# GuildOfWeavers/distaff

Measured on NVIDIA H100. Metric: prove ms for 2^20-step trace (default 120-bit ProofOptions), lower is better.
Workload: dtype u128 (128-bit prime field) + u32 (blake3)

## Files before the change

### distaff_b200/csrc/ntt.cu

```cuda
#define DG_MUL_CALL 1
#include "ntt_pass.cuh"

namespace dg {

PassKernel pass_kernel_inline(bool lane_major, int log_l, int rmax, int bt);
template <bool LM, int RMAX, int BT, int MINB> static PassKernel pass_kernel_t(int log_l) {
    switch (log_l) {
        case 1: return ntt_pass_kernel<1, LM, RMAX, BT, MINB, 0>;  case 2: return ntt_pass_kernel<2, LM, RMAX, BT, MINB, 0>;
        case 3: return ntt_pass_kernel<3, LM, RMAX, BT, MINB, 0>;  case 4: return ntt_pass_kernel<4, LM, RMAX, BT, MINB, 0>;
        case 5: return ntt_pass_kernel<5, LM, RMAX, BT, MINB, 0>;  case 6: return ntt_pass_kernel<6, LM, RMAX, BT, MINB, 0>;
        case 7: return ntt_pass_kernel<7, LM, RMAX, BT, MINB, 0>;  case 8: return ntt_pass_kernel<8, LM, RMAX, BT, MINB, 0>;
        case 9: return ntt_pass_kernel<9, LM, RMAX, BT, MINB, 0>;  case 10: return ntt_pass_kernel<10, LM, RMAX, BT, MINB, 0>;
    }
    throw Error(-1, "unsupported sub-transform size");
}

struct PassCfg { int rmax, bt, inl; };
struct NttConfig { PassCfg a, b, af; int tile_log; };
static PassCfg parse_cfg(const char *env, PassCfg d) {
    const char *e = getenv(env);
    if (e) { int r = 0, t = 0, i = 0; if (sscanf(e, "%d,%d,%d", &r, &t, &i) == 3) d = PassCfg{r, t, i}; }
    if (d.rmax < 2 || d.rmax > 4) d.rmax = 4;
    if (d.bt != 512 && d.bt != 1024) d.bt = 256;
    return d;
}
static const NttConfig &ntt_config() {
    static NttConfig cfg;
    static bool init = false;
    if (!init) {
        cfg.a = parse_cfg("DG_NTT_A", PassCfg{3, 512, 1});
        cfg.b = parse_cfg("DG_NTT_B", PassCfg{3, 512, 1});
        cfg.af = parse_cfg("DG_NTT_AF", PassCfg{2, 512, 1});
        const char *e = getenv("DG_NTT_TILE");
        cfg.tile_log = e ? atoi(e) : 12;
        if (cfg.tile_log < 12 || cfg.tile_log > 13) cfg.tile_log = 12;
        init = true;
    }
    return cfg;
}

static void launch_pass(Context &c, int log_l, PassGeom g, const fe *src, fe *dst, unsigned blocks_x, unsigned by, unsigned bz) {
    const int L = 1 << log_l, T = 1 << g.log_t;
    const size_t data = g.lane_major ? (size_t)T * (L + (L >> 3) + 1) : (size_t)L * T;
    const size_t smem = ((size_t)L + data) * sizeof(fe);
    const NttConfig &nc = ntt_config();
    const PassCfg cfg = g.lane_major ? nc.b : ((g.coset_on && !g.coset_fast) ? nc.af : nc.a);
    int rmax = cfg.rmax, bt = cfg.bt;
    PassKernel k = nullptr;
    if (cfg.inl) k = pass_kernel_inline(g.lane_major != 0, log_l, rmax, bt);
    if (!k) {
        const bool lm = g.lane_major != 0;
        if (bt == 1024) bt = 512;
        if (rmax == 4) { bt = 256; k = lm ? pass_kernel_t<true, 4, 256, 2>(log_l) : pass_kernel_t<false, 4, 256, 2>(log_l); }
        else if (rmax == 3 && bt == 512) k = lm ? pass_kernel_t<true, 3, 512, 2>(log_l) : pass_kernel_t<false, 3, 512, 2>(log_l);
        else if (rmax == 3) k = lm ? pass_kernel_t<true, 3, 256, 3>(log_l) : pass_kernel_t<false, 3, 256, 3>(log_l);
        else if (bt == 512) k = lm ? pass_kernel_t<true, 2, 512, 2>(log_l) : pass_kernel_t<false, 2, 512, 2>(log_l);
        else k = lm ? pass_kernel_t<true, 2, 256, 4>(log_l) : pass_kernel_t<false, 2, 256, 4>(log_l);
    }
    int threads = (L * T) >> (log_l < rmax ? log_l : rmax);
    if (threads > bt) threads = bt;
    if (threads < 32) threads = 32;
    set_func_smem(c, (const void *)k, 200 * 1024);
    DG_REQUIRE(by <= 65535 && bz <= 65535, "batch too large for one launch");
    k<<<dim3(blocks_x, by, bz), threads, smem, c.stream>>>(src, dst, g); c.launches++;
    DG_CUDA(cudaGetLastError());
}

static int lanes_log(int log_l, long long available) {
    int lt = 4;
    const int tile = 1 << ntt_config().tile_log;
    while ((1 << (log_l + lt)) > tile && lt > 0) lt--;
    while ((1LL << lt) > available && lt > 0) lt--;
    return lt;
}

static int split_passes(int log_n, int l[3]) {
    if (log_n <= MAX_LOG_L) { l[0] = log_n; return 1; }
    if (log_n <= 2 * MAX_LOG_L) { l[0] = (log_n + 1) / 2; l[1] = log_n / 2; return 2; }
    DG_REQUIRE(log_n <= 3 * MAX_LOG_L, "transform too large");
    l[0] = (log_n + 2) / 3; l[1] = (log_n + 1) / 3; l[2] = log_n / 3;
    return 3;
}

struct CosetSpec { bool on; int log_blowup; int fold; unsigned coset0; };

__global__ void lde_twiddle_fill_kernel(fe *table, TwiddleRef cw, int log_n, int log_r1, int log_b) {
    const unsigned long long i = (unsigned long long)blockIdx.x * blockDim.x + threadIdx.x;
    if (i >> (log_n + log_b)) return;
    const unsigned long long c = i >> log_n, pos = i & ((1ULL << log_n) - 1);
    const unsigned long long lane = pos & ((1ULL << log_r1) - 1), k = pos >> log_r1;
    table[i] = tw_lookup(cw, lane * ((k << log_b) + c));
}
static const fe *lde_twiddle_table(Context &c, int log_n, int log_b, int l0) {
    static long long cap = -1;
    if (cap < 0) { const char *e = getenv("DG_LDE_TW_MB"); cap = (e ? atoll(e) : 1024) << 20; }
    const size_t bytes = ((size_t)16 << (log_n + log_b));
    if ((long long)bytes > cap) return nullptr;
    const long long key = ((long long)log_n << 16) | (log_b << 8) | l0;
    auto it = c.lde_twiddles.find(key);
    if (it == c.lde_twiddles.end()) {
        DevBuf t;
        t.alloc(bytes, true);
        const unsigned long long cnt = 1ULL << (log_n + log_b);
        lde_twiddle_fill_kernel<<<(unsigned)((cnt + 255) / 256), 256, 0, c.stream>>>(t.as<fe>(), c.twiddle(log_n + log_b, false), log_n, log_n - l0, log_b);
        c.launches++;
        DG_CUDA(cudaGetLastError());
        it = c.lde_twiddles.emplace(key, std::move(t)).first;
    }
    return it->second.as<fe>();
}

static void run_transform(Context &c, const fe *src, fe *dst, int log_n, bool inverse, unsigned by, unsigned bz, long long src_stride_z,
                          long long dst_stride_y, long long dst_stride_z, CosetSpec cs) {
    int l[3];
    const int np = split_passes(log_n, l);
    const long long n = 1LL << log_n;
    fe scale = fe_make(1, 0);
    if (inverse) scale = host_inv(fe_make((unsigned long long)n, 0));

    PassGeom base;
    memset(&base, 0, sizeof base);
    if (cs.on) {
        base.coset_on = 1;
        base.fold = cs.fold;
        base.fold_stride = n;
        base.cw = c.twiddle(log_n + cs.log_blowup, false);
        base.log_blowup = cs.log_blowup;
        base.coset0 = cs.coset0;
        if (cs.fold == 1) {
            const int log_order = l[0] + cs.log_blowup;
            base.coset_fast = 1;
            base.cw_point = c.single_table(log_order);
            base.cw_point_mask = (1u << log_order) - 1u;
        }
    }

    fe *tmp = nullptr;
    long long tmp_stride_y = n, tmp_stride_z = n * by;
    if (np > 1) {
        c.ntt_tmp.ensure((size_t)n * by * bz * sizeof(fe), true);
        tmp = c.ntt_tmp.as<fe>();
// ... 31 lines not shown
        const long long N3 = 1LL << l[2];
        PassGeom g;
        memset(&g, 0, sizeof g);
        g.log_t = lanes_log(l[1], N3);
        g.num_tiles = (unsigned)(N3 >> g.log_t);
        g.in_point = N3; g.in_lane = 1; g.in_outer = R1; g.out_point = N3; g.out_lane = 1; g.out_outer = R1;
        g.in_batch_y = tmp_stride_y; g.in_batch_z = tmp_stride_z; g.out_batch_y = tmp_stride_y; g.out_batch_z = tmp_stride_z;
        g.lane_major = 0;
        g.tw_on = 1; g.tw = c.twiddle(log_n - l[0], inverse);
        g.roots = c.roots(l[1], inverse);
        launch_pass(c, l[1], g, tmp, tmp, (unsigned)(g.num_tiles * N1), by, bz);
    }
    {
        const int ll = l[np - 1];
        PassGeom g;
        memset(&g, 0, sizeof g);
        g.log_t = lanes_log(ll, N1);
        g.num_tiles = (unsigned)(N1 >> g.log_t);
        g.in_point = 1; g.in_lane = R1; g.in_outer = (np == 3) ? (1LL << ll) : 0;
        g.out_lane = 1; g.out_outer = (np == 3) ? N1 : 0; g.out_point = N1 * N2;
        g.in_batch_y = tmp_stride_y; g.in_batch_z = tmp_stride_z; g.out_batch_y = dst_stride_y; g.out_batch_z = dst_stride_z;
        g.lane_major = 1; g.tw_on = 0;
        g.has_scale = inverse; g.scale = scale;
        g.roots = c.roots(ll, inverse);
        launch_pass(c, ll, g, tmp, dst, (unsigned)(g.num_tiles * N2), by, bz);
    }
}

void ntt_batch(Context &c, const fe *src, fe *dst, int log_n, int batch, size_t src_stride, size_t dst_stride, bool inverse) {
    DG_REQUIRE(log_n >= 1 && log_n <= 30, "log_n out of range");
    const size_t n = (size_t)1 << log_n;
    size_t max_chunk = std::max<size_t>(1, ((size_t)1 << 30) / (n * sizeof(fe)));
    if (max_chunk > 65535) max_chunk = 65535;
    for (size_t b0 = 0; b0 < (size_t)batch; b0 += max_chunk) {
        size_t nb = std::min(max_chunk, (size_t)batch - b0);
        run_transform(c, src + b0 * src_stride, dst + b0 * dst_stride, log_n, inverse, 1, (unsigned)nb, (long long)src_stride, 0,
                      (long long)dst_stride, CosetSpec{false, 0, 1, 0});
    }
}

__global__ void __launch_bounds__(256) prefold8_kernel(const fe *__restrict__ src, fe *__restrict__ dst, int log_n, int log_b, const fe *__restrict__ zeta,
                                                       TwiddleRef twN, fe w8, fe w8_2, fe w8_3) {
    const unsigned long long n = 1ULL << log_n;
    const unsigned long long t = (unsigned long long)blockIdx.x * blockDim.x + threadIdx.x;
    if (t >> (log_n + log_b - 3)) return;
    const unsigned long long j = t & (n - 1);
    const unsigned r = (unsigned)(t >> log_n);
    const unsigned bmask = (1u << log_b) - 1u, step = 1u << (log_b - 3);
    fe x[8];
#pragma unroll
    for (int f = 0; f < 8; f++) x[f] = src[j + (unsigned long long)f * n];
    if (r) {
#pragma unroll
        for (int f = 1; f < 8; f++) x[f] = fe_mul(x[f], zeta[(r * (unsigned)f) & bmask]);
    }
    fe u[4], v[4];
    const fe wp[4] = {fe_make(1, 0), w8, w8_2, w8_3};
#pragma unroll
    for (int i = 0; i < 4; i++) {
        u[i] = fe_add(x[i], x[i + 4]);
        v[i] = fe_sub(x[i], x[i + 4]);
        if (i) v[i] = fe_mul(v[i], wp[i]);
    }
    fe X[8];
    {
        fe p0 = fe_add(u[0], u[2]), p1 = fe_add(u[1], u[3]), q0 = fe_sub(u[0], u[2]), q1 = fe_mul(fe_sub(u[1], u[3]), w8_2);
        X[0] = fe_add(p0, p1); X[4] = fe_sub(p0, p1); X[2] = fe_add(q0, q1); X[6] = fe_sub(q0, q1);
        p0 = fe_add(v[0], v[2]); p1 = fe_add(v[1], v[3]); q0 = fe_sub(v[0], v[2]); q1 = fe_mul(fe_sub(v[1], v[3]), w8_2);
        X[1] = fe_add(p0, p1); X[5] = fe_sub(p0, p1); X[3] = fe_add(q0, q1); X[7] = fe_sub(q0, q1);
    }
    fe cur = tw_lookup(twN, (unsigned long long)r * j);
    const fe rho = tw_lookup(twN, (unsigned long long)step * j);
#pragma unroll
    for (int q = 0; q < 8; q++) {
        dst[((unsigned long long)(step * (unsigned)q + r) << log_n) + j] = fe_mul(X[q], cur);
        if (q < 7) cur = fe_mul(cur, rho);
    }
}

void lde_batch(Context &c, const fe *src, fe *dst, int log_n, int log_blowup, int fold, int batch, size_t src_stride, size_t dst_stride,
               unsigned coset0, unsigned ncosets) {
    DG_REQUIRE(log_n >= 1 && log_n + log_blowup <= 30, "LDE domain too large");
    const size_t n = (size_t)1 << log_n;
    const unsigned cosets = ncosets ? ncosets : (1u << log_blowup);
    DG_REQUIRE(coset0 + cosets <= (1u << log_blowup), "coset range out of bounds");
    static int prefold = -1;
    if (prefold < 0) { const char *e = getenv("DG_LDE_PREFOLD"); prefold = e ? atoi(e) : 1; }
    if (prefold && fold == 8 && batch == 1 && cosets == (1u << log_blowup) && log_blowup >= 3 && log_blowup <= 8) {
        DevBuf pre((size_t)n * cosets * sizeof(fe));
        const fe w8 = host_root_of_unity(3), w8_2 = fe_mul(w8, w8);
        const unsigned long long threads = (unsigned long long)n << (log_blowup - 3);
        prefold8_kernel<<<(unsigned)((threads + 255) / 256), 256, 0, c.stream>>>(src, pre.as<fe>(), log_n, log_blowup, c.single_table(log_blowup),
                                                                                 c.twiddle(log_n + log_blowup, false), w8, w8_2, fe_mul(w8_2, w8)); c.launches++;
        DG_CUDA(cudaGetLastError());
        ntt_batch(c, pre.as<fe>(), dst, log_n, (int)cosets, n, n, false);
        return;
    }
    static size_t scratch_cap = 0;
    if (!scratch_cap) { const char *e = getenv("DG_NTT_SCRATCH_MB"); scratch_cap = (size_t)(e ? atoll(e) : 4096) << 20; }
    size_t max_chunk = std::max<size_t>(1, scratch_cap / (n * cosets * sizeof(fe)));
    if (max_chunk > 65535) max_chunk = 65535;
    for (size_t b0 = 0; b0 < (size_t)batch; b0 += max_chunk) {
        size_t nb = std::min(max_chunk, (size_t)batch - b0);
        run_transform(c, src + b0 * src_stride, dst + b0 * dst_stride, log_n, false, cosets, (unsigned)nb, (long long)src_stride,
                      (long long)n, (long long)dst_stride, CosetSpec{true, log_blowup, fold, coset0});
    }
}

}
```

### distaff_b200/csrc/ntt_inl.cu

```cuda
#include "ntt_pass.cuh"

namespace dg {

template <bool LM, int RMAX, int BT, int MINB> static PassKernel inl_t(int log_l) {
    switch (log_l) {
        case 8: return ntt_pass_kernel<8, LM, RMAX, BT, MINB, 1>;
        case 9: return ntt_pass_kernel<9, LM, RMAX, BT, MINB, 1>;
        case 10: return ntt_pass_kernel<10, LM, RMAX, BT, MINB, 1>;
    }
    return nullptr;
}

PassKernel pass_kernel_inline(bool lm, int log_l, int rmax, int bt) {
    if (rmax == 3 && bt == 1024) return lm ? inl_t<true, 3, 1024, 1>(log_l) : inl_t<false, 3, 1024, 1>(log_l);
    if (rmax == 3 && bt == 512) return lm ? inl_t<true, 3, 512, 2>(log_l) : inl_t<false, 3, 512, 2>(log_l);
    if (rmax == 3) return lm ? inl_t<true, 3, 256, 3>(log_l) : inl_t<false, 3, 256, 3>(log_l);
    if (rmax == 2 && bt == 512) return lm ? inl_t<true, 2, 512, 2>(log_l) : inl_t<false, 2, 512, 2>(log_l);
    if (rmax == 2) return lm ? inl_t<true, 2, 256, 4>(log_l) : inl_t<false, 2, 256, 4>(log_l);
    return nullptr;
}

}
```

### distaff_b200/csrc/ntt_pass.cuh

```cuda
#pragma once
#include "common.cuh"

namespace dg {

struct PassGeom {
    int log_t;
    unsigned num_tiles;
    long long in_outer, in_lane, in_point;
    long long out_outer, out_lane, out_point;
    long long in_batch_y, out_batch_y, in_batch_z, out_batch_z;
    int lane_major;
    int tw_on;
    TwiddleRef tw;
    int has_scale;
    fe scale;
    int coset_on;
    int fold;
    long long fold_stride;
    TwiddleRef cw;
    int coset_fast;
    const fe *cw_point;
    unsigned cw_point_mask;
    const fe *tw_full;
    long long tw_full_stride;
    int log_blowup;
    unsigned coset0;
    const fe *roots;
};

__device__ __forceinline__ fe tw_lookup(const TwiddleRef &t, unsigned long long e) {
    unsigned ee = (unsigned)e & t.mask;
    fe a = t.lo[ee & ((1u << t.lo_bits) - 1u)];
    fe b = t.hi[ee >> t.lo_bits];
    return fe_mul(a, b);
}

template <int LOG_L, int S0, int RHO>
__device__ __forceinline__ void dif_regs(fe *x, const fe *s_tw, int g_lo) {
    constexpr int L = 1 << LOG_L, R = 1 << RHO;
    constexpr int LOG_SP = LOG_L - S0 - RHO;
#pragma unroll
    for (int u = 0; u < RHO; u++) {
        const int hr = R >> (u + 1);
        const int st = S0 + u;
        const fe *W = s_tw + (L - (L >> st));
#pragma unroll
        for (int i = 0; i < R; i++) {
            if ((i & hr) == 0) {
                fe a = x[i], b = x[i + hr];
                x[i] = fe_add(a, b);
                fe d = fe_sub(a, b);
                if (st != LOG_L - 1 && !(LOG_SP == 0 && (i & (hr - 1)) == 0)) d = fe_mul(d, W[g_lo + ((i & (hr - 1)) << LOG_SP)]);
                x[i + hr] = d;
            }
        }
    }
}

template <int LOG_L, bool LANE_MAJOR>
__device__ __forceinline__ int sidx(int pos, int t, int T) {
    constexpr int L = 1 << LOG_L;
    constexpr int LS = L + (L >> 3) + 1;
    return LANE_MAJOR ? (t * LS + pos + (pos >> 3)) : (pos * T + t);
}

template <int LOG_L, int S0, int RHO, bool FIRST, bool LAST, bool LANE_MAJOR>
__device__ __forceinline__ void ntt_round(const fe *__restrict__ src, fe *__restrict__ dst, fe *s_data, const fe *s_tw, const PassGeom &g,
                                          unsigned tile, long long in_base) {
    constexpr int L = 1 << LOG_L, R = 1 << RHO;
    constexpr int LOG_B = LOG_L - S0, LOG_SP = LOG_B - RHO;
    constexpr int N_GLO = 1 << LOG_SP, N_GHI = 1 << S0;
    const int T = 1 << g.log_t;
    const int units = (L >> RHO) * T;
    for (int u = threadIdx.x; u < units; u += blockDim.x) {
        int t, g_lo, g_hi;
        if (!LANE_MAJOR || LAST) {
            t = u & (T - 1);
            const int rest = u >> g.log_t;
            g_lo = rest & (N_GLO - 1);
            g_hi = rest >> LOG_SP;
        } else {
            g_lo = u & (N_GLO - 1);
            const int rest = u >> LOG_SP;
            g_hi = rest & (N_GHI - 1);
            t = rest >> S0;
        }
        const int gbase = (g_hi << LOG_B) + g_lo;
        fe x[R];
#pragma unroll
        for (int m = 0; m < R; m++) {
            const int pos = gbase + (m << LOG_SP);
            if (FIRST) {
                const long long j = in_base + (long long)t * g.in_lane + (long long)pos * g.in_point;
                if (g.coset_fast) {
                    x[m] = fe_mul(src[j], g.cw_point[((g.coset0 + (unsigned)blockIdx.y) * (unsigned)pos) & g.cw_point_mask]);
                } else if (g.coset_on) {
                    const unsigned long long c = g.coset0 + blockIdx.y;
                    const fe u = tw_lookup(g.cw, c * (unsigned long long)g.fold_stride);
                    fe v = src[j + (long long)(g.fold - 1) * g.fold_stride];
                    for (int f = g.fold - 2; f >= 0; f--) v = fe_add(fe_mul(v, u), src[j + (long long)f * g.fold_stride]);
                    x[m] = fe_mul(v, tw_lookup(g.cw, c * (unsigned long long)j));
                } else {
                    x[m] = src[j];
                }
            } else {
                x[m] = s_data[sidx<LOG_L, LANE_MAJOR>(pos, t, T)];
            }
        }
        dif_regs<LOG_L, S0, RHO>(x, s_tw, g_lo);
#pragma unroll
        for (int m = 0; m < R; m++) {
            const int pos = gbase + (m << LOG_SP);
            if (LAST) {
                const unsigned k = __brev((unsigned)pos) >> (32 - LOG_L);
                fe v = x[m];
                if (g.coset_fast && g.tw_on) {
                    if (g.tw_full)
                        v = fe_mul(v, g.tw_full[(long long)(g.coset0 + blockIdx.y) * g.tw_full_stride + (long long)(tile * T + t) * g.out_lane + (long long)k * g.out_point]);
                    else
                        v = fe_mul(v, tw_lookup(g.cw, (unsigned long long)(tile * T + t) * (((unsigned long long)k << g.log_blowup) + g.coset0 + blockIdx.y)));
                }
                else if (g.tw_on) v = fe_mul(v, tw_lookup(g.tw, (unsigned long long)(tile * T + t) * k));
                if (g.has_scale) v = fe_mul(v, g.scale);
                dst[(long long)t * g.out_lane + (long long)k * g.out_point] = v;
            } else {
                s_data[sidx<LOG_L, LANE_MAJOR>(pos, t, T)] = x[m];
            }
        }
    }
}

template <int LOG_L, int RMAX, int S0, bool LANE_MAJOR>
__device__ __forceinline__ void ntt_rounds(const fe *__restrict__ src, fe *__restrict__ dst, fe *s_data, const fe *s_tw, const PassGeom &g,
                                           unsigned tile, long long in_base) {
    constexpr int REM = LOG_L - S0, LEFT = (REM + RMAX - 1) / RMAX, RHO = (REM + LEFT - 1) / LEFT;
    ntt_round<LOG_L, S0, RHO, S0 == 0, S0 + RHO == LOG_L, LANE_MAJOR>(src, dst, s_data, s_tw, g, tile, in_base);
    if constexpr (S0 + RHO < LOG_L) {
        __syncthreads();
        ntt_rounds<LOG_L, RMAX, S0 + RHO, LANE_MAJOR>(src, dst, s_data, s_tw, g, tile, in_base);
    }
}

template <int LOG_L, bool LANE_MAJOR, int RMAX, int BT, int MINB, int TAG>
__global__ void __launch_bounds__(BT, MINB) ntt_pass_kernel(const fe *__restrict__ src, fe *__restrict__ dst, const PassGeom g) {
    extern __shared__ __align__(16) unsigned char smem_raw[];
    constexpr int L = 1 << LOG_L;
    fe *s_tw = reinterpret_cast<fe *>(smem_raw);
    fe *s_data = s_tw + L;
    const int T = 1 << g.log_t;
    const unsigned tile = blockIdx.x % g.num_tiles, outer = blockIdx.x / g.num_tiles;
    const long long in_base = (long long)outer * g.in_outer + (long long)tile * T * g.in_lane;
    src += (long long)blockIdx.y * g.in_batch_y + (long long)blockIdx.z * g.in_batch_z;
    dst += (long long)blockIdx.y * g.out_batch_y + (long long)blockIdx.z * g.out_batch_z + (long long)outer * g.out_outer +
           (long long)tile * T * g.out_lane;
    for (int i = threadIdx.x; i < L - 1; i += blockDim.x) s_tw[i] = g.roots[i];
    if (g.tw_full) {
        const fe *tb = g.tw_full + (long long)(g.coset0 + blockIdx.y) * g.tw_full_stride + (long long)tile * T * g.out_lane;
        for (int k = threadIdx.x; k < L; k += blockDim.x)
            asm volatile("prefetch.global.L2 [%0];" :: "l"(tb + (long long)k * g.out_point));
    }
    __syncthreads();
    ntt_rounds<LOG_L, RMAX, 0, LANE_MAJOR>(src, dst, s_data, s_tw, g, tile, in_base);
}

typedef void (*PassKernel)(const fe *, fe *, const PassGeom);

}
```

### distaff_b200/csrc/prover.cu

```cuda
#include "prover.h"
#include "air.h"
#include "host_fs.h"
#include "poly.h"
#include "shard.h"
#include <array>
#include <atomic>
#include <memory>
#include <thread>

namespace dg {

namespace {

struct StageClock {
    cudaStream_t s;
    cudaEvent_t ev[10];
    explicit StageClock(cudaStream_t stream) : s(stream) { for (auto &e : ev) DG_CUDA(cudaEventCreate(&e)); }
    ~StageClock() { for (auto &e : ev) cudaEventDestroy(e); }
    void mark(int i) { DG_CUDA(cudaEventRecord(ev[i], s)); }
    float between(int a, int b) { float ms = 0; cudaEventElapsedTime(&ms, ev[a], ev[b]); return ms; }
};

struct SubClock {
    bool on;
    cudaStream_t s;
    std::vector<std::pair<std::string, cudaEvent_t>> marks;
    explicit SubClock(cudaStream_t stream) : on(getenv("DG_SUBSTAGE") != nullptr), s(stream) {}
    void mark(const char *name) {
        if (!on) return;
        cudaEvent_t e;
        cudaEventCreate(&e);
        cudaEventRecord(e, s);
        marks.emplace_back(name, e);
    }
    void report(int rank) {
        if (!on) return;
        cudaStreamSynchronize(s);
        std::string line = "SUBSTAGE rank " + std::to_string(rank) + ":";
        for (size_t i = 1; i < marks.size(); i++) {
            float ms = 0;
            cudaEventElapsedTime(&ms, marks[i - 1].second, marks[i].second);
            char buf[96];
            snprintf(buf, sizeof buf, " %s=%.3f", marks[i].first.c_str(), ms);
            line += buf;
        }
        if (rank == 0 || atoi(getenv("DG_SUBSTAGE")) >= 2) fprintf(stderr, "%s\n", line.c_str());
        for (auto &m : marks) cudaEventDestroy(m.second);
        marks.clear();
    }
};

void d2h(Context &c, void *dst, const void *src, size_t bytes) {
    DG_CUDA(cudaMemcpyAsync(dst, src, bytes, cudaMemcpyDeviceToHost, c.stream));
    DG_CUDA(cudaStreamSynchronize(c.stream));
}
void h2d(Context &c, void *dst, const void *src, size_t bytes) {
    DG_CUDA(cudaMemcpyAsync(dst, src, bytes, cudaMemcpyHostToDevice, c.stream));
}

void debug_dump(Context &c, const char *name, const void *dev, size_t bytes) {
    const char *dir = getenv("DG_DEBUG_DUMP");
    if (!dir) return;
    std::vector<uint8_t> host(bytes);
    d2h(c, host.data(), dev, bytes);
    std::string path = std::string(dir) + "/" + name + ".bin";
    FILE *f = fopen(path.c_str(), "wb");
    if (!f) return;
    fwrite(host.data(), 1, bytes, f);
    fclose(f);
}

void debug_dump_host(const char *name, const void *host, size_t bytes) {
    const char *dir = getenv("DG_DEBUG_DUMP");
    if (!dir) return;
    std::string path = std::string(dir) + "/" + name + ".bin";
    FILE *f = fopen(path.c_str(), "wb");
    if (!f) return;
    fwrite(host, 1, bytes, f);
    fclose(f);
}


void write_digest_vec(fs::ByteWriter &w, const std::vector<Digest> &v) {
    w.u64(v.size());
    for (auto &d : v) w.raw(d.data(), 32);
}
void write_digest_vv(fs::ByteWriter &w, const std::vector<std::vector<Digest>> &v) {
    w.u64(v.size());
    for (auto &x : v) write_digest_vec(w, x);
}
void write_felt_vec(fs::ByteWriter &w, const std::vector<fe> &v) {
    w.u64(v.size());
    for (auto &x : v) w.felt(x);
}

int ilog2(uint64_t v) { int l = 0; while ((1ULL << l) < v) l++; return l; }

struct FriLayerDev {
    DevBuf leaves, nodes, folded;
    const fe *vals;
    Layout layout;
    bool sharded = false;
    ShardedTree tree;
    Digest root;
};

}

class TraceUploader {
public:
    static const int WORKERS = 4, SLOTS = 2;
    TraceUploader(Context &c, fe *d_regs, const uint8_t *const *host_cols, int w, uint64_t n, const std::vector<int> &bounds)
        : c_(c), w_(w), bounds_(bounds), nchunks_((int)bounds.size() - 1), col_bytes_(n * 16), done_(nchunks_, nullptr), recorded_(nchunks_) {
        for (auto &r : recorded_) r.store(0);
        for (auto &e : done_) DG_CUDA(cudaEventCreateWithFlags(&e, cudaEventDisableTiming));
        cudaEvent_t ready;
        DG_CUDA(cudaEventCreateWithFlags(&ready, cudaEventDisableTiming));
        DG_CUDA(cudaEventRecord(ready, c.stream));
        cudaPointerAttributes attr;
        bool pinned = cudaPointerGetAttributes(&attr, host_cols[0]) == cudaSuccess && attr.type != cudaMemoryTypeUnregistered;
        cudaGetLastError();
        if (getenv("DG_NO_STAGING")) pinned = true;
        if (pinned) {
            DG_CUDA(cudaStreamWaitEvent(c.copy_stream, ready, 0));
            for (int i = 0; i < nchunks_; i++) {
                for (int j = bounds_[i]; j < bounds_[i + 1]; j++)
                    DG_CUDA(cudaMemcpyAsync(d_regs + (size_t)j * n, host_cols[j], col_bytes_, cudaMemcpyHostToDevice, c.copy_stream));
                DG_CUDA(cudaEventRecord(done_[i], c.copy_stream));
                recorded_[i].store(1);
            }
        } else {
            c.staging.ensure((size_t)WORKERS * SLOTS * col_bytes_);
            for (int t = 0; t < WORKERS; t++) {
                if (!c.staging_streams[t]) DG_CUDA(cudaStreamCreateWithFlags(&c.staging_streams[t], cudaStreamNonBlocking));
                DG_CUDA(cudaStreamWaitEvent(c.staging_streams[t], ready, 0));
            }
            const int dev = c.device;
            for (int t = 0; t < WORKERS; t++)
                workers_.emplace_back([this, t, dev, d_regs, host_cols, n]() {
                    cudaSetDevice(dev);
                    cudaStream_t st = c_.staging_streams[t];
                    cudaEvent_t slot_free[SLOTS] = {nullptr, nullptr};
                    int use = 0;
                    for (int i = t; i < nchunks_ && !failed_.load(); i += WORKERS) {
                        for (int j = bounds_[i]; j < bounds_[i + 1]; j++, use++) {
                            const int s = use % SLOTS;
                            uint8_t *slot = (uint8_t *)c_.staging.p + ((size_t)t * SLOTS + s) * col_bytes_;
                            if (slot_free[s]) cudaEventSynchronize(slot_free[s]);
                            else cudaEventCreateWithFlags(&slot_free[s], cudaEventDisableTiming);
                            memcpy(slot, host_cols[j], col_bytes_);
                            if (cudaMemcpyAsync(d_regs + (size_t)j * n, slot, col_bytes_, cudaMemcpyHostToDevice, st) != cudaSuccess) failed_.store(true);
                            cudaEventRecord(slot_free[s], st);
                        }
                        if (cudaEventRecord(done_[i], st) != cudaSuccess) failed_.store(true);
                        recorded_[i].store(1);
                    }
                    for (int i = t; i < nchunks_; i += WORKERS) recorded_[i].store(1);
                    cudaStreamSynchronize(st);
                    for (auto &e : slot_free) if (e) cudaEventDestroy(e);
                });
        }
        cudaEventDestroy(ready);
    }
    void wait_chunk(int i) {
        while (!recorded_[i].load()) std::this_thread::yield();
        if (failed_.load()) throw Error(DG_ERR_CUDA, "host trace upload failed");
        DG_CUDA(cudaStreamWaitEvent(c_.stream, done_[i], 0));
    }
    int chunks() const { return nchunks_; }
    ~TraceUploader() {
        failed_.store(true);
        for (auto &t : workers_) t.join();
        cudaStreamSynchronize(c_.copy_stream);
        for (auto &e : done_) if (e) cudaEventDestroy(e);
    }
private:
    Context &c_;
    int w_;
    std::vector<int> bounds_;
    int nchunks_;
    size_t col_bytes_;
    std::vector<cudaEvent_t> done_;
    std::vector<std::atomic<int>> recorded_;
    std::atomic<bool> failed_{false};
    std::vector<std::thread> workers_;
};

static Proof *prove_core(Context &c, fe *d_regs, const uint8_t *const *host_cols, uint32_t width, uint64_t length, uint32_t ctx_depth,
                         uint32_t loop_depth, const uint8_t *inputs16, uint32_t n_inputs, const uint8_t *outputs16, uint32_t n_outputs,
                         const dg_options_t &opt, dg_prove_stats_t *stats) {
    const uint64_t n = length, b = opt.extension_factor;
    DG_REQUIRE(opt.hash_id == 0, "unsupported hash function (only blake3 is serialisable, options.rs:107)");
    DG_REQUIRE(b >= 16 && b <= 256 && (b & (b - 1)) == 0, "extension_factor must be a power of 2 between 16 and 256");
    DG_REQUIRE(opt.num_queries > 0 && opt.num_queries <= 128, "num_queries must be in 1..128");
    DG_REQUIRE(opt.grinding_factor <= 32, "grinding factor cannot be greater than 32");
    DG_REQUIRE(n >= 16 && (n & (n - 1)) == 0, "execution trace length must be a power of 2 and at least 16");
    DG_REQUIRE(ctx_depth <= 16, "context depth cannot be greater than 16");
    DG_REQUIRE(loop_depth <= 8, "loop depth cannot be greater than 8");
    DG_REQUIRE(width < 128, "execution trace cannot have more than 128 registers");
    DG_REQUIRE(width > 15 + ctx_depth + loop_depth, "user stack must consist of at least one register");
    DG_REQUIRE(n_inputs <= 8 && n_outputs <= 8, "cannot have more than 8 public inputs / outputs");
    const int w = (int)width, log_n = ilog2(n), log_b = ilog2(b), log_N = log_n + log_b;
    DG_REQUIRE(log_N <= 30, "LDE domain too large");
    const uint64_t N = n * b, E = n * 8;
    const int stack_depth = w - 15 - (int)ctx_depth - (int)loop_depth;
    DG_REQUIRE(stack_depth <= 32, "stack depth cannot be greater than 32");
    std::vector<fe> inputs(n_inputs), outputs(n_outputs);
    if (n_inputs) memcpy(inputs.data(), inputs16, n_inputs * 16);
    if (n_outputs) memcpy(outputs.data(), outputs16, n_outputs * 16);

    ArenaScope arena_scope;
    StageClock clk(c.stream);
    SubClock sub(c.stream);
    if (sub.on) c.mark = [&sub](const char *name) { sub.mark(name); }; else c.mark = nullptr;
    struct MarkReset { Context &c; ~MarkReset() { c.mark = nullptr; } } mark_reset{c};
    const unsigned long long launches0 = c.launches;
    Proof *proof = new Proof();
    std::unique_ptr<Proof> guard(proof);

    const int G = c.world, g = c.rank;
    int log_g = 0;
    while ((1 << log_g) < G) log_g++;
    DG_REQUIRE((b >> log_g) >= 4 && G <= 8, "extension factor too small for this many GPUs (need >= 4 cosets per rank)");
    const int log_nc = log_b - log_g;
    const uint64_t nc = 1ULL << log_nc, N_loc = n * nc;
    const unsigned c0 = (unsigned)(g * nc);

    clk.mark(0);
    sub.mark("start");
    const int cpr = (w + G - 1) / G;
    auto col_count = [&](int r) { return w / G + (r < w % G ? 1 : 0); };
    auto col_start = [&](int r) { return r * (w / G) + std::min(r, w % G); };
    DevBuf polys((size_t)w * n * 16), ext((size_t)w * N_loc * 16);
    if (G == 1) {
        if (!host_cols) {
            ntt_batch(c, d_regs, polys.as<fe>(), log_n, w, n, n, true);
            lde_batch(c, polys.as<fe>(), ext.as<fe>(), log_n, log_b, 1, w, n, N_loc, c0, (unsigned)nc);
        } else {
            const int chunk = (int)std::max<uint64_t>(1, std::min<uint64_t>(w, ((uint64_t)1 << 26) / (n * 16)));
            std::vector<int> bounds = {0};
            for (int step = 1; bounds.back() < w; step = std::min(chunk, step * 2)) bounds.push_back(std::min(w, bounds.back() + step));
            TraceUploader up(c, d_regs, host_cols, w, n, bounds);
            for (int i = 0; i < up.chunks(); i++) {
                const int j0 = bounds[i], cols = bounds[i + 1] - j0;
                up.wait_chunk(i);
                ntt_batch(c, d_regs + (size_t)j0 * n, polys.as<fe>() + (size_t)j0 * n, log_n, cols, n, n, true);
                lde_batch(c, polys.as<fe>() + (size_t)j0 * n, ext.as<fe>() + (size_t)j0 * N_loc, log_n, log_b, 1, cols, n, N_loc, c0, (unsigned)nc);
            }
        }
    } else {
        const int j0 = col_start(g), mine = col_count(g);
        DevBuf own((size_t)cpr * n * 16), slots((size_t)cpr * G * n * 16);
        if (mine > 0) {
            if (host_cols) {
                std::vector<int> bounds(mine + 1);
                for (int i = 0; i <= mine; i++) bounds[i] = i;
                TraceUploader up(c, d_regs + (size_t)j0 * n, host_cols + j0, mine, n, bounds);
                for (int i = 0; i < up.chunks(); i++) {
                    up.wait_chunk(i);
                    ntt_batch(c, d_regs + (size_t)(j0 + i) * n, own.as<fe>() + (size_t)i * n, log_n, 1, n, n, true);
                }
            } else {
                ntt_batch(c, d_regs + (size_t)j0 * n, own.as<fe>(), log_n, mine, n, n, true);
            }
        }
    sub.mark("1.intt");
        cudaEvent_t ev_own, ev_all;
        DG_CUDA(cudaEventCreateWithFlags(&ev_own, cudaEventDisableTiming));
        DG_CUDA(cudaEventCreateWithFlags(&ev_all, cudaEventDisableTiming));
        DG_CUDA(cudaEventRecord(ev_own, c.stream));
        DG_CUDA(cudaStreamWaitEvent(c.comm_stream, ev_own, 0));
        comm_all_gather(c, own.p, slots.p, (size_t)cpr * n * 16, c.comm_stream);
        for (int r = 0; r < G; r++)
            if (col_count(r) > 0)
                DG_CUDA(cudaMemcpyAsync(polys.as<fe>() + (size_t)col_start(r) * n, slots.as<fe>() + (size_t)r * cpr * n, (size_t)col_count(r) * n * 16,
                                        cudaMemcpyDeviceToDevice, c.comm_stream));
        DG_CUDA(cudaEventRecord(ev_all, c.comm_stream));
        if (mine > 0) lde_batch(c, own.as<fe>(), ext.as<fe>() + (size_t)j0 * N_loc, log_n, log_b, 1, mine, n, N_loc, c0, (unsigned)nc);
    sub.mark("1.lde_own");
        DG_CUDA(cudaStreamWaitEvent(c.stream, ev_all, 0));
        if (j0 > 0) lde_batch(c, polys.as<fe>(), ext.as<fe>(), log_n, log_b, 1, j0, n, N_loc, c0, (unsigned)nc);
        if (j0 + mine < w)
            lde_batch(c, polys.as<fe>() + (size_t)(j0 + mine) * n, ext.as<fe>() + (size_t)(j0 + mine) * N_loc, log_n, log_b, 1, w - j0 - mine, n, N_loc, c0,
                      (unsigned)nc);
        cudaEventDestroy(ev_own);
        cudaEventDestroy(ev_all);
    }

    clk.mark(1);
    sub.mark("1.lde");
    DevBuf t_leaves(N_loc * 32);
    hash_trace_rows(c, ext.as<fe>(), t_leaves.p, w, log_n, log_nc);
    sub.mark("2.hash_rows");
    ShardedTree t_tree;
    t_tree.build(c, t_leaves.p, n, log_nc);
    memcpy(proof->trace_root, t_tree.root.data(), 32);

    clk.mark(2);
    sub.mark("2.tree");
    fe last_row[3];
    if (host_cols) {
        for (int j = 0; j < 3; j++) memcpy(&last_row[j], host_cols[j] + (n - 1) * 16, 16);
    } else {
        DevBuf d_last(48);
        for (int j = 0; j < 3; j++) DG_CUDA(cudaMemcpyAsync((uint8_t *)d_last.p + 16 * j, d_regs + (size_t)j * n + (n - 1), 16, cudaMemcpyDeviceToDevice, c.stream));
        d2h(c, last_row, d_last.p, 48);
    }
    const fe op_count = last_row[0];
    const fe program_hash[2] = {last_row[1], last_row[2]};
    fs::ConstraintCoefficients cc = fs::draw_constraint_coefficients(proof->trace_root, ctx_depth, loop_depth, stack_depth, inputs, outputs,
                                                                      op_count, program_hash);
    DevBuf &d_periodic = c.d_periodic;
    if (!d_periodic.p) {
        std::vector<fe> per = fs::periodic_tables();
        d_periodic.alloc(per.size() * 16, true);
        h2d(c, d_periodic.p, per.data(), per.size() * 16);
        DG_CUDA(cudaStreamSynchronize(c.stream));
    }
    const size_t T = cc.coefA.size(), nb = cc.bAi.size();
    DevBuf d_coef((2 * T + 4 * nb) * 16), d_violation(4);
    {
        std::vector<fe> pack;
        pack.insert(pack.end(), cc.coefA.begin(), cc.coefA.end());
        pack.insert(pack.end(), cc.coefB.begin(), cc.coefB.end());
        pack.insert(pack.end(), cc.bAi.begin(), cc.bAi.end());
        pack.insert(pack.end(), cc.bBi.begin(), cc.bBi.end());
        pack.insert(pack.end(), cc.bAf.begin(), cc.bAf.end());
        pack.insert(pack.end(), cc.bBf.begin(), cc.bBf.end());
        h2d(c, d_coef.p, pack.data(), pack.size() * 16);
        DG_CUDA(cudaStreamSynchronize(c.stream));
    }
    DG_CUDA(cudaMemsetAsync(d_violation.p, 0, 4, c.stream));
    DevBuf evals(3 * E * 16);
    {
        const int num_c8 = 8 >> log_g;
        const uint64_t E_loc = n * num_c8;
        DevBuf evals_loc(E_loc * 16), gathered(E * 16);
        AirParams P;
        memset(&P, 0, sizeof P);
        P.w = w; P.ctx_depth = ctx_depth; P.loop_depth = loop_depth; P.stack_depth = stack_depth;
        P.cl = std::max<int>(ctx_depth, 1); P.ll = std::max<int>(loop_depth, 1); P.sl = std::max(stack_depth, 8);
        P.log_n = log_n; P.log_blowup = log_b;
        P.ext = ext.as<fe>(); P.col_stride = N_loc;
        P.c8_base = g * num_c8; P.num_c8 = num_c8;
        P.t_ev = evals_loc.as<fe>();
        P.periodic = d_periodic.as<fe>();
        const fe *base = d_coef.as<fe>();
        P.coefA = base; P.coefB = base + T;
        P.twN = c.twiddle(log_N, false);
        static const int GROUP_DEG[6] = {2, 3, 4, 6, 7, 8};
        for (int gi = 0; gi < 6; gi++) P.inc[gi] = (8 * n - 1) - (n - 1) * GROUP_DEG[gi];
        P.violation = d_violation.as<unsigned>();
    sub.mark("3.setup");
        launch_constraint_eval(c, P);
    sub.mark("3.eval");
        comm_all_reduce_max_u32(c, d_violation.as<unsigned>(), 1);
        unsigned violation = 0;
        d2h(c, &violation, d_violation.p, 4);
        if (violation) throw Error(DG_ERR_UNSATISFIED, "transition constraints at step " + std::to_string(violation - 1) + " were not satisfied");
    sub.mark("3.violation_sync");
        ntt_batch(c, evals_loc.as<fe>(), evals_loc.as<fe>(), log_n, num_c8, n, n, true);
        comm_all_gather(c, evals_loc.as<fe>(), gathered.as<fe>(), E_loc * 16);
    sub.mark("3.intt+gather");
        coset_interp_finish(c, gathered.as<fe>(), evals.as<fe>() + 2 * E, log_n);
        boundary_coeffs(c, polys.as<fe>(), n, (int)nb, base + 2 * T, cc.KiA, cc.KiB, cc.KfA, cc.KfB, evals.as<fe>(), evals.as<fe>() + E);
    }
    debug_dump(c, "t_coeffs", evals.as<fe>() + 2 * E, E * 16);
// ... 316 lines not shown
```

Before: 134.2.

## Specialize NTT pass kernels by pass kind and reuse trace for coset zero

Replaces runtime branching on coset, twiddle and scale flags inside the NTT pass kernel with a compile-time PassKind template parameter, so each variant compiles only the multiply path it needs. It also changes the default radix for strided and contiguous passes from 3 to 2. When the LDE covers coset 0, the original trace columns are copied into the extension buffer instead of being recomputed by an NTT, which removes one coset of transforms. The cost is more kernel instantiations, and the copy assumes coset 0 of the extension equals the trace in natural order.

```diff
diff --git a/distaff_b200/csrc/ntt.cu b/distaff_b200/csrc/ntt.cu
--- a/distaff_b200/csrc/ntt.cu
+++ b/distaff_b200/csrc/ntt.cu
@@ -3,16 +3,20 @@
 
 namespace dg {
 
-PassKernel pass_kernel_inline(bool lane_major, int log_l, int rmax, int bt);
-template <bool LM, int RMAX, int BT, int MINB> static PassKernel pass_kernel_t(int log_l) {
-    switch (log_l) {
-        case 1: return ntt_pass_kernel<1, LM, RMAX, BT, MINB, 0>;  case 2: return ntt_pass_kernel<2, LM, RMAX, BT, MINB, 0>;
-        case 3: return ntt_pass_kernel<3, LM, RMAX, BT, MINB, 0>;  case 4: return ntt_pass_kernel<4, LM, RMAX, BT, MINB, 0>;
-        case 5: return ntt_pass_kernel<5, LM, RMAX, BT, MINB, 0>;  case 6: return ntt_pass_kernel<6, LM, RMAX, BT, MINB, 0>;
-        case 7: return ntt_pass_kernel<7, LM, RMAX, BT, MINB, 0>;  case 8: return ntt_pass_kernel<8, LM, RMAX, BT, MINB, 0>;
-        case 9: return ntt_pass_kernel<9, LM, RMAX, BT, MINB, 0>;  case 10: return ntt_pass_kernel<10, LM, RMAX, BT, MINB, 0>;
-    }
-    throw Error(-1, "unsupported sub-transform size");
+PassKernel pass_kernel_inline(int kind, int log_l, int rmax, int bt);
+
+static int pass_kind(const PassGeom &g) {
+    if (!g.lane_major) {
+        DG_REQUIRE(g.tw_on && !g.has_scale, "strided NTT pass without inter-pass twiddle");
+        if (g.coset_fast) return g.tw_full ? PK_COSET_TWFULL : PK_COSET_TW;
+        return g.coset_on ? PK_FOLD_TW : PK_TW;
+    }
+    DG_REQUIRE(!g.tw_on, "contiguous NTT pass with inter-pass twiddle");
+    if (g.coset_on) {
+        DG_REQUIRE(!g.has_scale, "scaled coset transform");
+        return g.coset_fast ? PK_COSET_ONE : PK_FOLD_ONE;
+    }
+    return g.has_scale ? PK_LAST_SCALE : PK_LAST;
 }
 
 struct PassCfg { int rmax, bt, inl; };
@@ -28,8 +32,8 @@
     static NttConfig cfg;
     static bool init = false;
     if (!init) {
-        cfg.a = parse_cfg("DG_NTT_A", PassCfg{3, 512, 1});
-        cfg.b = parse_cfg("DG_NTT_B", PassCfg{3, 512, 1});
+        cfg.a = parse_cfg("DG_NTT_A", PassCfg{2, 512, 1});
+        cfg.b = parse_cfg("DG_NTT_B", PassCfg{2, 512, 1});
         cfg.af = parse_cfg("DG_NTT_AF", PassCfg{2, 512, 1});
         const char *e = getenv("DG_NTT_TILE");
         cfg.tile_log = e ? atoi(e) : 12;
@@ -45,18 +49,19 @@
     const size_t smem = ((size_t)L + data) * sizeof(fe);
     const NttConfig &nc = ntt_config();
     const PassCfg cfg = g.lane_major ? nc.b : ((g.coset_on && !g.coset_fast) ? nc.af : nc.a);
+    const int kind = pass_kind(g);
     int rmax = cfg.rmax, bt = cfg.bt;
     PassKernel k = nullptr;
-    if (cfg.inl) k = pass_kernel_inline(g.lane_major != 0, log_l, rmax, bt);
+    if (cfg.inl) k = pass_kernel_inline(kind, log_l, rmax, bt);
     if (!k) {
-        const bool lm = g.lane_major != 0;
         if (bt == 1024) bt = 512;
-        if (rmax == 4) { bt = 256; k = lm ? pass_kernel_t<true, 4, 256, 2>(log_l) : pass_kernel_t<false, 4, 256, 2>(log_l); }
-        else if (rmax == 3 && bt == 512) k = lm ? pass_kernel_t<true, 3, 512, 2>(log_l) : pass_kernel_t<false, 3, 512, 2>(log_l);
-        else if (rmax == 3) k = lm ? pass_kernel_t<true, 3, 256, 3>(log_l) : pass_kernel_t<false, 3, 256, 3>(log_l);
-        else if (bt == 512) k = lm ? pass_kernel_t<true, 2, 512, 2>(log_l) : pass_kernel_t<false, 2, 512, 2>(log_l);
-        else k = lm ? pass_kernel_t<true, 2, 256, 4>(log_l) : pass_kernel_t<false, 2, 256, 4>(log_l);
-    }
+        if (rmax == 4) { bt = 256; k = pass_kernel_of<4, 256, 2, 0, 1, MAX_LOG_L>(kind, log_l); }
+        else if (rmax == 3 && bt == 512) k = pass_kernel_of<3, 512, 2, 0, 1, MAX_LOG_L>(kind, log_l);
+        else if (rmax == 3) k = pass_kernel_of<3, 256, 3, 0, 1, MAX_LOG_L>(kind, log_l);
+        else if (bt == 512) k = pass_kernel_of<2, 512, 2, 0, 1, MAX_LOG_L>(kind, log_l);
+        else k = pass_kernel_of<2, 256, 4, 0, 1, MAX_LOG_L>(kind, log_l);
+    }
+    DG_REQUIRE(k, "unsupported sub-transform size");
     int threads = (L * T) >> (log_l < rmax ? log_l : rmax);
     if (threads > bt) threads = bt;
     if (threads < 32) threads = 32;
@@ -254,8 +259,9 @@
                unsigned coset0, unsigned ncosets) {
     DG_REQUIRE(log_n >= 1 && log_n + log_blowup <= 30, "LDE domain too large");
     const size_t n = (size_t)1 << log_n;
-    const unsigned cosets = ncosets ? ncosets : (1u << log_blowup);
-    DG_REQUIRE(coset0 + cosets <= (1u << log_blowup), "coset range out of bounds");
+    DG_REQUIRE(log_blowup >= 0 && log_blowup <= 16 && fold >= 1, "bad LDE shape");
+    const unsigned b = 1u << log_blowup, cosets = ncosets ? ncosets : b;
+    DG_REQUIRE(coset0 < b && cosets <= b - coset0, "coset range out of bounds");
     static int prefold = -1;
     if (prefold < 0) { const char *e = getenv("DG_LDE_PREFOLD"); prefold = e ? atoi(e) : 1; }
     if (prefold && fold == 8 && batch == 1 && cosets == (1u << log_blowup) && log_blowup >= 3 && log_blowup <= 8) {
diff --git a/distaff_b200/csrc/ntt_inl.cu b/distaff_b200/csrc/ntt_inl.cu
--- a/distaff_b200/csrc/ntt_inl.cu
+++ b/distaff_b200/csrc/ntt_inl.cu
@@ -2,21 +2,12 @@
 
 namespace dg {
 
-template <bool LM, int RMAX, int BT, int MINB> static PassKernel inl_t(int log_l) {
-    switch (log_l) {
-        case 8: return ntt_pass_kernel<8, LM, RMAX, BT, MINB, 1>;
-        case 9: return ntt_pass_kernel<9, LM, RMAX, BT, MINB, 1>;
-        case 10: return ntt_pass_kernel<10, LM, RMAX, BT, MINB, 1>;
-    }
-    return nullptr;
-}
-
-PassKernel pass_kernel_inline(bool lm, int log_l, int rmax, int bt) {
-    if (rmax == 3 && bt == 1024) return lm ? inl_t<true, 3, 1024, 1>(log_l) : inl_t<false, 3, 1024, 1>(log_l);
-    if (rmax == 3 && bt == 512) return lm ? inl_t<true, 3, 512, 2>(log_l) : inl_t<false, 3, 512, 2>(log_l);
-    if (rmax == 3) return lm ? inl_t<true, 3, 256, 3>(log_l) : inl_t<false, 3, 256, 3>(log_l);
-    if (rmax == 2 && bt == 512) return lm ? inl_t<true, 2, 512, 2>(log_l) : inl_t<false, 2, 512, 2>(log_l);
-    if (rmax == 2) return lm ? inl_t<true, 2, 256, 4>(log_l) : inl_t<false, 2, 256, 4>(log_l);
+PassKernel pass_kernel_inline(int kind, int log_l, int rmax, int bt) {
+    if (rmax == 3 && bt == 1024) return pass_kernel_of<3, 1024, 1, 1, 8, 10>(kind, log_l);
+    if (rmax == 3 && bt == 512) return pass_kernel_of<3, 512, 2, 1, 8, 10>(kind, log_l);
+    if (rmax == 3) return pass_kernel_of<3, 256, 3, 1, 8, 10>(kind, log_l);
+    if (rmax == 2 && bt == 512) return pass_kernel_of<2, 512, 2, 1, 8, 10>(kind, log_l);
+    if (rmax == 2) return pass_kernel_of<2, 256, 4, 1, 8, 10>(kind, log_l);
     return nullptr;
 }
 
diff --git a/distaff_b200/csrc/ntt_pass.cuh b/distaff_b200/csrc/ntt_pass.cuh
--- a/distaff_b200/csrc/ntt_pass.cuh
+++ b/distaff_b200/csrc/ntt_pass.cuh
@@ -2,6 +2,21 @@
 #include "common.cuh"
 
 namespace dg {
+
+enum PassKind {
+    PK_TW,
+    PK_COSET_TWFULL,
+    PK_COSET_TW,
+    PK_FOLD_TW,
+    PK_LAST,
+    PK_LAST_SCALE,
+    PK_COSET_ONE,
+    PK_FOLD_ONE,
+    PK_COUNT
+};
+__host__ __device__ constexpr bool pk_lane_major(int k) { return k >= PK_LAST; }
+__host__ __device__ constexpr bool pk_coset_in(int k) { return k == PK_COSET_TWFULL || k == PK_COSET_TW || k == PK_COSET_ONE; }
+__host__ __device__ constexpr bool pk_fold_in(int k) { return k == PK_FOLD_TW || k == PK_FOLD_ONE; }
 
 struct PassGeom {
     int log_t;
@@ -11,14 +26,14 @@
     long long in_batch_y, out_batch_y, in_batch_z, out_batch_z;
     int lane_major;
     int tw_on;
+    int has_scale;
+    int coset_on;
+    int coset_fast;
     TwiddleRef tw;
-    int has_scale;
     fe scale;
-    int coset_on;
     int fold;
     long long fold_stride;
     TwiddleRef cw;
-    int coset_fast;
     const fe *cw_point;
     unsigned cw_point_mask;
     const fe *tw_full;
@@ -28,11 +43,19 @@
     const fe *roots;
 };
 
+__device__ __forceinline__ fe ntt_mul(fe a, fe b) {
+#if defined(__CUDA_ARCH__) && !defined(DG_MUL_CALL)
+    return ptx::fe_mul_v4t<false>(a, b);
+#else
+    return fe_mul(a, b);
+#endif
+}
+
 __device__ __forceinline__ fe tw_lookup(const TwiddleRef &t, unsigned long long e) {
     unsigned ee = (unsigned)e & t.mask;
     fe a = t.lo[ee & ((1u << t.lo_bits) - 1u)];
     fe b = t.hi[ee >> t.lo_bits];
-    return fe_mul(a, b);
+    return ntt_mul(a, b);
 }
 
 template <int LOG_L, int S0, int RHO>
@@ -50,7 +73,7 @@
                 fe a = x[i], b = x[i + hr];
                 x[i] = fe_add(a, b);
                 fe d = fe_sub(a, b);
-                if (st != LOG_L - 1 && !(LOG_SP == 0 && (i & (hr - 1)) == 0)) d = fe_mul(d, W[g_lo + ((i & (hr - 1)) << LOG_SP)]);
+                if (st != LOG_L - 1 && !(LOG_SP == 0 && (i & (hr - 1)) == 0)) d = ntt_mul(d, W[g_lo + ((i & (hr - 1)) << LOG_SP)]);
                 x[i + hr] = d;
             }
         }
@@ -64,9 +87,10 @@
     return LANE_MAJOR ? (t * LS + pos + (pos >> 3)) : (pos * T + t);
 }
 
-template <int LOG_L, int S0, int RHO, bool FIRST, bool LAST, bool LANE_MAJOR>
+template <int LOG_L, int S0, int RHO, bool FIRST, bool LAST, int KIND>
 __device__ __forceinline__ void ntt_round(const fe *__restrict__ src, fe *__restrict__ dst, fe *s_data, const fe *s_tw, const PassGeom &g,
                                           unsigned tile, long long in_base) {
+    constexpr bool LANE_MAJOR = pk_lane_major(KIND);
     constexpr int L = 1 << LOG_L, R = 1 << RHO;
     constexpr int LOG_B = LOG_L - S0, LOG_SP = LOG_B - RHO;
     constexpr int N_GLO = 1 << LOG_SP, N_GHI = 1 << S0;
@@ -92,14 +116,14 @@
             const int pos = gbase + (m << LOG_SP);
             if (FIRST) {
                 const long long j = in_base + (long long)t * g.in_lane + (long long)pos * g.in_point;
-                if (g.coset_fast) {
-                    x[m] = fe_mul(src[j], g.cw_point[((g.coset0 + (unsigned)blockIdx.y) * (unsigned)pos) & g.cw_point_mask]);
-                } else if (g.coset_on) {
+                if (pk_coset_in(KIND)) {
+                    x[m] = ntt_mul(src[j], g.cw_point[((g.coset0 + (unsigned)blockIdx.y) * (unsigned)pos) & g.cw_point_mask]);
+                } else if (pk_fold_in(KIND)) {
                     const unsigned long long c = g.coset0 + blockIdx.y;
                     const fe u = tw_lookup(g.cw, c * (unsigned long long)g.fold_stride);
                     fe v = src[j + (long long)(g.fold - 1) * g.fold_stride];
-                    for (int f = g.fold - 2; f >= 0; f--) v = fe_add(fe_mul(v, u), src[j + (long long)f * g.fold_stride]);
-                    x[m] = fe_mul(v, tw_lookup(g.cw, c * (unsigned long long)j));
+                    for (int f = g.fold - 2; f >= 0; f--) v = fe_add(ntt_mul(v, u), src[j + (long long)f * g.fold_stride]);
+                    x[m] = ntt_mul(v, tw_lookup(g.cw, c * (unsigned long long)j));
                 } else {
                     x[m] = src[j];
                 }
@@ -114,14 +138,14 @@
             if (LAST) {
                 const unsigned k = __brev((unsigned)pos) >> (32 - LOG_L);
                 fe v = x[m];
-                if (g.coset_fast && g.tw_on) {
-                    if (g.tw_full)
-                        v = fe_mul(v, g.tw_full[(long long)(g.coset0 + blockIdx.y) * g.tw_full_stride + (long long)(tile * T + t) * g.out_lane + (long long)k * g.out_point]);
-                    else
-                        v = fe_mul(v, tw_lookup(g.cw, (unsigned long long)(tile * T + t) * (((unsigned long long)k << g.log_blowup) + g.coset0 + blockIdx.y)));
-                }
-                else if (g.tw_on) v = fe_mul(v, tw_lookup(g.tw, (unsigned long long)(tile * T + t) * k));
-                if (g.has_scale) v = fe_mul(v, g.scale);
+                if (KIND == PK_COSET_TWFULL)
+                    v = ntt_mul(v, g.tw_full[(long long)(g.coset0 + blockIdx.y) * g.tw_full_stride + (long long)(tile * T + t) * g.out_lane + (long long)k * g.out_point]);
+                else if (KIND == PK_COSET_TW)
+                    v = ntt_mul(v, tw_lookup(g.cw, (unsigned long long)(tile * T + t) * (((unsigned long long)k << g.log_blowup) + g.coset0 + blockIdx.y)));
+                else if (KIND == PK_TW || KIND == PK_FOLD_TW)
+                    v = ntt_mul(v, tw_lookup(g.tw, (unsigned long long)(tile * T + t) * k));
+                else if (KIND == PK_LAST_SCALE)
+                    v = ntt_mul(v, g.scale);
                 dst[(long long)t * g.out_lane + (long long)k * g.out_point] = v;
             } else {
                 s_data[sidx<LOG_L, LANE_MAJOR>(pos, t, T)] = x[m];
@@ -130,18 +154,18 @@
     }
 }
 
-template <int LOG_L, int RMAX, int S0, bool LANE_MAJOR>
+template <int LOG_L, int RMAX, int S0, int KIND>
 __device__ __forceinline__ void ntt_rounds(const fe *__restrict__ src, fe *__restrict__ dst, fe *s_data, const fe *s_tw, const PassGeom &g,
                                            unsigned tile, long long in_base) {
     constexpr int REM = LOG_L - S0, LEFT = (REM + RMAX - 1) / RMAX, RHO = (REM + LEFT - 1) / LEFT;
-    ntt_round<LOG_L, S0, RHO, S0 == 0, S0 + RHO == LOG_L, LANE_MAJOR>(src, dst, s_data, s_tw, g, tile, in_base);
+    ntt_round<LOG_L, S0, RHO, S0 == 0, S0 + RHO == LOG_L, KIND>(src, dst, s_data, s_tw, g, tile, in_base);
     if constexpr (S0 + RHO < LOG_L) {
         __syncthreads();
-        ntt_rounds<LOG_L, RMAX, S0 + RHO, LANE_MAJOR>(src, dst, s_data, s_tw, g, tile, in_base);
-    }
-}
-
-template <int LOG_L, bool LANE_MAJOR, int RMAX, int BT, int MINB, int TAG>
+        ntt_rounds<LOG_L, RMAX, S0 + RHO, KIND>(src, dst, s_data, s_tw, g, tile, in_base);
+    }
+}
+
+template <int LOG_L, int KIND, int RMAX, int BT, int MINB, int TAG>
 __global__ void __launch_bounds__(BT, MINB) ntt_pass_kernel(const fe *__restrict__ src, fe *__restrict__ dst, const PassGeom g) {
     extern __shared__ __align__(16) unsigned char smem_raw[];
     constexpr int L = 1 << LOG_L;
@@ -154,15 +178,33 @@
     dst += (long long)blockIdx.y * g.out_batch_y + (long long)blockIdx.z * g.out_batch_z + (long long)outer * g.out_outer +
            (long long)tile * T * g.out_lane;
     for (int i = threadIdx.x; i < L - 1; i += blockDim.x) s_tw[i] = g.roots[i];
-    if (g.tw_full) {
+    if (KIND == PK_COSET_TWFULL) {
         const fe *tb = g.tw_full + (long long)(g.coset0 + blockIdx.y) * g.tw_full_stride + (long long)tile * T * g.out_lane;
         for (int k = threadIdx.x; k < L; k += blockDim.x)
             asm volatile("prefetch.global.L2 [%0];" :: "l"(tb + (long long)k * g.out_point));
     }
     __syncthreads();
-    ntt_rounds<LOG_L, RMAX, 0, LANE_MAJOR>(src, dst, s_data, s_tw, g, tile, in_base);
+    ntt_rounds<LOG_L, RMAX, 0, KIND>(src, dst, s_data, s_tw, g, tile, in_base);
 }
 
 typedef void (*PassKernel)(const fe *, fe *, const PassGeom);
 
-}
+template <int KIND, int RMAX, int BT, int MINB, int TAG, int LO, int HI> PassKernel pass_kernel_sized(int log_l) {
+    if constexpr (LO > HI) return nullptr;
+    else return log_l == LO ? ntt_pass_kernel<LO, KIND, RMAX, BT, MINB, TAG> : pass_kernel_sized<KIND, RMAX, BT, MINB, TAG, LO + 1, HI>(log_l);
+}
+template <int RMAX, int BT, int MINB, int TAG, int LO, int HI> PassKernel pass_kernel_of(int kind, int log_l) {
+    switch (kind) {
+        case PK_TW: return pass_kernel_sized<PK_TW, RMAX, BT, MINB, TAG, LO, HI>(log_l);
+        case PK_COSET_TWFULL: return pass_kernel_sized<PK_COSET_TWFULL, RMAX, BT, MINB, TAG, LO, HI>(log_l);
+        case PK_COSET_TW: return pass_kernel_sized<PK_COSET_TW, RMAX, BT, MINB, TAG, LO, HI>(log_l);
+        case PK_FOLD_TW: return pass_kernel_sized<PK_FOLD_TW, RMAX, BT, MINB, TAG, LO, HI>(log_l);
+        case PK_LAST: return pass_kernel_sized<PK_LAST, RMAX, BT, MINB, TAG, LO, HI>(log_l);
+        case PK_LAST_SCALE: return pass_kernel_sized<PK_LAST_SCALE, RMAX, BT, MINB, TAG, LO, HI>(log_l);
+        case PK_COSET_ONE: return pass_kernel_sized<PK_COSET_ONE, RMAX, BT, MINB, TAG, LO, HI>(log_l);
+        case PK_FOLD_ONE: return pass_kernel_sized<PK_FOLD_ONE, RMAX, BT, MINB, TAG, LO, HI>(log_l);
+    }
+    return nullptr;
+}
+
+}
diff --git a/distaff_b200/csrc/prover.cu b/distaff_b200/csrc/prover.cu
--- a/distaff_b200/csrc/prover.cu
+++ b/distaff_b200/csrc/prover.cu
@@ -95,6 +95,18 @@
 }
 
 int ilog2(uint64_t v) { int l = 0; while ((1ULL << l) < v) l++; return l; }
+
+void extend_trace_columns(Context &c, const fe *polys, const fe *regs, fe *ext, int cols, int log_n, int log_b, uint64_t N_loc, unsigned c0,
+                          unsigned nc) {
+    const size_t n = (size_t)1 << log_n;
+    if (c0 != 0 || !regs) {
+        lde_batch(c, polys, ext, log_n, log_b, 1, cols, n, N_loc, c0, nc);
+        return;
+    }
+    DG_REQUIRE(nc >= 2, "coset range too small");
+    lde_batch(c, polys, ext + n, log_n, log_b, 1, cols, n, N_loc, 1, nc - 1);
+    DG_CUDA(cudaMemcpy2DAsync(ext, N_loc * sizeof(fe), regs, n * sizeof(fe), n * sizeof(fe), cols, cudaMemcpyDeviceToDevice, c.stream));
+}
 
 struct FriLayerDev {
     DevBuf leaves, nodes, folded;
@@ -235,7 +247,7 @@
     if (G == 1) {
         if (!host_cols) {
             ntt_batch(c, d_regs, polys.as<fe>(), log_n, w, n, n, true);
-            lde_batch(c, polys.as<fe>(), ext.as<fe>(), log_n, log_b, 1, w, n, N_loc, c0, (unsigned)nc);
+            extend_trace_columns(c, polys.as<fe>(), d_regs, ext.as<fe>(), w, log_n, log_b, N_loc, c0, (unsigned)nc);
         } else {
             const int chunk = (int)std::max<uint64_t>(1, std::min<uint64_t>(w, ((uint64_t)1 << 26) / (n * 16)));
             std::vector<int> bounds = {0};
@@ -245,7 +257,8 @@
                 const int j0 = bounds[i], cols = bounds[i + 1] - j0;
                 up.wait_chunk(i);
                 ntt_batch(c, d_regs + (size_t)j0 * n, polys.as<fe>() + (size_t)j0 * n, log_n, cols, n, n, true);
-                lde_batch(c, polys.as<fe>() + (size_t)j0 * n, ext.as<fe>() + (size_t)j0 * N_loc, log_n, log_b, 1, cols, n, N_loc, c0, (unsigned)nc);
+                extend_trace_columns(c, polys.as<fe>() + (size_t)j0 * n, d_regs + (size_t)j0 * n, ext.as<fe>() + (size_t)j0 * N_loc, cols, log_n, log_b, N_loc,
+                                     c0, (unsigned)nc);
             }
         }
     } else {
@@ -276,13 +289,14 @@
                 DG_CUDA(cudaMemcpyAsync(polys.as<fe>() + (size_t)col_start(r) * n, slots.as<fe>() + (size_t)r * cpr * n, (size_t)col_count(r) * n * 16,
                                         cudaMemcpyDeviceToDevice, c.comm_stream));
         DG_CUDA(cudaEventRecord(ev_all, c.comm_stream));
-        if (mine > 0) lde_batch(c, own.as<fe>(), ext.as<fe>() + (size_t)j0 * N_loc, log_n, log_b, 1, mine, n, N_loc, c0, (unsigned)nc);
+        if (mine > 0)
+            extend_trace_columns(c, own.as<fe>(), d_regs + (size_t)j0 * n, ext.as<fe>() + (size_t)j0 * N_loc, mine, log_n, log_b, N_loc, c0, (unsigned)nc);
     sub.mark("1.lde_own");
         DG_CUDA(cudaStreamWaitEvent(c.stream, ev_all, 0));
-        if (j0 > 0) lde_batch(c, polys.as<fe>(), ext.as<fe>(), log_n, log_b, 1, j0, n, N_loc, c0, (unsigned)nc);
+        if (j0 > 0) extend_trace_columns(c, polys.as<fe>(), host_cols ? nullptr : d_regs, ext.as<fe>(), j0, log_n, log_b, N_loc, c0, (unsigned)nc);
         if (j0 + mine < w)
-            lde_batch(c, polys.as<fe>() + (size_t)(j0 + mine) * n, ext.as<fe>() + (size_t)(j0 + mine) * N_loc, log_n, log_b, 1, w - j0 - mine, n, N_loc, c0,
-                      (unsigned)nc);
+            extend_trace_columns(c, polys.as<fe>() + (size_t)(j0 + mine) * n, host_cols ? nullptr : d_regs + (size_t)(j0 + mine) * n,
+                                 ext.as<fe>() + (size_t)(j0 + mine) * N_loc, w - j0 - mine, log_n, log_b, N_loc, c0, (unsigned)nc);
         cudaEventDestroy(ev_own);
         cudaEventDestroy(ev_all);
     }
```

New measurement: 121.6 (median of 6 runs). 1.1x faster.
